# brocksam/pycollo

Hardware: AMD Instinct MI355X
Metric: NLP-callback evals/sec (g + jac_g + hess) (higher is better)
Workload: dtype f64; 1 GPU; hypersensitive, 1 phase, 2000 mesh sections x 6 Lobatto nodes = 10001 collocation nodes; num_x=20003, num_c=10001, nnz_jac=140003, nnz_hess=20002, tiles=167, threads_per_block=64, waves_per_tile=4, launches_per_eval=1, lds_bytes_per_workgroup=24144, launch_thread_cpu=199, pin_survived_hip_init=True

## Files before the change

### __graft_entry__.py

```python
from __future__ import annotations

import os
import subprocess
import sys

ROOT = os.path.dirname(os.path.abspath(__file__))
if ROOT not in sys.path:
    sys.path.insert(0, ROOT)

CSRC = os.path.join(ROOT, "pycollo_amd", "csrc")
LIB = os.path.join(ROOT, "pycollo_amd", "libpycollo_amd.so")


def _run(cmd):
    res = subprocess.run(cmd, capture_output=True, text=True)
    if res.returncode != 0:
        raise RuntimeError(f"{' '.join(cmd)} failed:\n{res.stdout[-2000:]}\n{res.stderr[-4000:]}")


def _stale(target, sources):
    if not os.path.exists(target):
        return True
    t = os.path.getmtime(target)
    return any(os.path.getmtime(s) > t for s in sources)


def build_library(force: bool = False) -> str:
    srcs = [os.path.join(CSRC, f) for f in ("pc_engine.hip", "pc_kkt.hip", "pc_host.hpp", "pc_ipm.hpp", "pc_kkt_cr.hpp", "pc_kkt_shape.hpp", "pc_eval_shape.hpp", "pc_eval_launch.hpp", "pc_pattern.hpp", "pc_desc.hpp", "pc_args.h", "pc_deriv.hpp", "pc_deriv_check.hpp",
                                           "pc_solution_plan.hpp", "pc_costate_plan.hpp", "pc_propagate_plan.hpp",
                                           "pc_solution_host.hpp")]
    srcs.append(os.path.join(ROOT, "include", "pycollo_amd.h"))
    if force or _stale(LIB, srcs):
        hipcc = "/opt/rocm/bin/hipcc" if os.path.exists("/opt/rocm/bin/hipcc") else "hipcc"
        _run([hipcc, "--offload-arch=gfx950", "-O2", "-ffp-contract=off", "-fPIC", "-shared", "-std=c++17", "-o", LIB + ".tmp",
              os.path.join(CSRC, "pc_engine.hip"), os.path.join(CSRC, "pc_kkt.hip")])
        os.replace(LIB + ".tmp", LIB)
    return LIB


PREBUILD = [
    ("brachistochrone", {}, (0,)), ("brachistochrone", {}, (4,)),
    ("hypersensitive", {}, (0,)), ("hypersensitive", {}, (6,)), ("hypersensitive", {}, (5,)), ("hypersensitive", {}, (4,)),
    ("hypersensitive", {}, (2,)), ("hypersensitive", {}, (8,)), ("hypersensitive", {}, (3,)),
    ("hypersensitive", {"fixed_control": 0.0}, (0,)),
    ("cart_pole", {}, (0,)), ("cart_pole", {}, (4,)), ("cart_pole", {}, (5,)),
    ("shuttle", {}, (0,)), ("shuttle", {}, (4,)), ("shuttle", {}, (5,)), ("shuttle", {}, (6,)),
    ("double_pendulum", {}, (0,)), ("double_pendulum", {}, (4,)),
    ("two_phase_transfer", {}, (0, 0)), ("two_phase_transfer", {}, (3, 4)), ("two_phase_transfer", {}, (4, 5)),
    ("two_phase_transfer", {}, (2, 2)), ("two_phase_transfer", {}, (3, 3)), ("two_phase_transfer", {}, (4, 4)),
    ("time_coupled_transfer", {}, (0, 0)), ("time_coupled_transfer", {}, (4, 4)),
    ("time_coupled_transfer", {}, (3, 3)), ("time_coupled_transfer", {}, (3, 4)),
# ... 121 lines not shown
```

### include/pycollo_amd.h

```cpp
#ifndef PYCOLLO_AMD_H
#define PYCOLLO_AMD_H

#include <stdint.h>

#ifdef __cplusplus
extern "C" {
#endif

typedef struct pc_handle pc_handle;

enum { PC_PT_Y0 = 0, PC_PT_YF = 1, PC_PT_Q = 2, PC_PT_T0 = 3, PC_PT_TF = 4, PC_PT_S = 5 };

typedef struct {
  int32_t n_y, n_u, n_q, n_p;
  int32_t t0_free, tF_free;
  double t0_fixed, tF_fixed;
  int32_t K;
  const int32_t* n_k;
  const double* h_k;
  int32_t n_jac;
  const int32_t* jac_row;
  const int32_t* jac_col;
  int32_t n_hess;
  const int32_t* hess_row;
// ... 40 lines not shown
  int32_t device;
  int32_t threads_per_block;
  int32_t two_wave_occupancy;
  int32_t plan_only;
} pc_problem_desc;

typedef struct {
  int32_t n, m;
  int64_t nnz_jac, nnz_hess;
  int64_t algorithmic_bytes;
  int32_t n_tiles_total, threads_per_block;
  int32_t lds_bytes_max, n_launches;
  int32_t waves_per_tile;
  int32_t last_launch;
} pc_info;

#define PC_LAUNCH_RESIDENT 1
#define PC_LAUNCH_TAIL_BIG 2
#define PC_LAUNCH_MERGED 4
#define PC_LAUNCH_TAIL_BLOCKS_SHIFT 4
#define PC_LAUNCH_TAIL_BLOCKS_MASK 7
#define PC_LAUNCH_TAIL_WAVES_SHIFT 8
#define PC_LAUNCH_TAIL_WAVES_MASK 15

const char* pc_last_error(void);

int pc_create(const pc_problem_desc* desc, pc_handle** out);
void pc_destroy(pc_handle* h);
int pc_get_info(const pc_handle* h, pc_info* info);

int pc_sizes(const pc_handle* h, int32_t* n, int32_t* m, int64_t* nnz_jac, int64_t* nnz_hess);
int pc_jac_structure(const pc_handle* h, int32_t* iRow, int32_t* jCol);
int pc_hess_structure(const pc_handle* h, int32_t* iRow, int32_t* jCol);

int pc_set_scaling(pc_handle* h, const double* V_ocp, const double* r_ocp, const double* W_ocp, double w_J);

int pc_eval_f(pc_handle* h, const double* x, int new_x, double* f);
int pc_eval_grad_f(pc_handle* h, const double* x, int new_x, double* grad);
int pc_eval_g(pc_handle* h, const double* x, int new_x, double* g);
int pc_eval_jac_g(pc_handle* h, const double* x, int new_x, double* values);
int pc_eval_h(pc_handle* h, const double* x, int new_x, double obj_factor, const double* lambda,
              int new_lambda, double* values);
int pc_eval_all(pc_handle* h, const double* x, double obj_factor, const double* lambda, double* g,
                double* jac, double* hess);
int pc_ipopt_eval_f(int n, double* x, int new_x, double* obj_value, void* user_data);
int pc_ipopt_eval_grad_f(int n, double* x, int new_x, double* grad_f, void* user_data);
// ... 207 lines not shown
```

### pycollo_amd/csrc/pc_engine.hip

```cpp
#include <hip/hip_runtime.h>

#include <chrono>
#include <cmath>
#include <cstdio>
#include <cstdlib>
#include <cstring>
#include <map>
#include <memory>
#include <string>
#include <vector>

#include "../../include/pycollo_amd.h"
#include "pc_args.h"
#include "pc_host.hpp"
#include "pc_pattern.hpp"
#include "pc_desc.hpp"
#include "pc_eval_shape.hpp"
#include "pc_eval_launch.hpp"
#include "pc_deriv.hpp"
#include "pc_solution_plan.hpp"

struct pc_deriv_dev;
struct pc_kkt;

namespace {

thread_local std::string g_err;

void set_err(const std::string& s) { g_err = s; }

struct PhaseDev {
  DevBuf<int32_t> tile_k0, tile_n0, sec_s;
  DevBuf<double> sec_h, scal, partials, tab;
  DevBuf<int64_t> sec_E, hslot0, hslotN, hsum_slot;
  DevBuf<int32_t> hsum_local;
  DevBuf<unsigned long long> gran;
  hipFunction_t fn = nullptr;
};

__global__ void row_norms_kernel(const int64_t* __restrict__ indptr, const double* __restrict__ val,
                                 double* __restrict__ out, int64_t m) {
// ... 36 lines not shown
}

struct pc_handle : pce::Shape {
  pcp::Problem Q;
  int device = -1;
  bool scaling_set = false;
  std::vector<double> qa, qw;
  hipStream_t stream = nullptr;
  hipModule_t module = nullptr;
  std::vector<hipModule_t> more_modules;
  hipFunction_t fn[pcl::N_KERNELS] = {};
  pcl::Have have;
  pcl::Range rg[PC_MAX_PHASES];
  pcl::Scaling scal;
  pcl::Blocks blocks;
  bool blocks_dirty = true;
  DevBuf<char> d_phase_args;
  DevBuf<PcTileRec> d_trec;
  std::vector<std::unique_ptr<PhaseDev>> pd;
  DevBuf<double> d_qa, d_pointV, d_pointr, d_Wend, d_norms;
  DevBuf<double> d_in, d_out;
  PinBuf<double> h_in, h_out;
  int host_mode = 0;
  hipEvent_t ev_small = nullptr, ev_G = nullptr;
  bool x_valid = false;
  bool fc_valid = false;
  bool small_synced = false, G_synced = false;
  bool prefetch_jac = true;
  bool G_copied = false;
  DevBuf<int64_t> d_point_x, d_tail_owned, d_pt_hslot, d_g_indptr;
  DevBuf<int32_t> d_pt_hlocal;
  DevBuf<unsigned long long> d_erec;
  DevBuf<int64_t> d_rec_slot;
  DevBuf<int32_t> d_rec_term;
  PinBuf<unsigned> h_timeout;
  int spin_us = 500;
  DevBuf<unsigned long long> d_hb_gran;
  PinBuf<double> h_norms;
  std::vector<double> V_ocp, r_ocp, W_ocp;
  int n_launches = 0;
  int last_launch = 0;
  mutable std::shared_ptr<pcd::Plan> deriv_plan;
  std::shared_ptr<pc_deriv_dev> deriv_dev;
};

namespace {

// ... 179 lines not shown
  if (!new_x && h->x_valid) return;
  if (!x) throw std::runtime_error("null x");
  if (x != h->h_in.p) std::memcpy(h->h_in.p, x, h->Q.num_x * sizeof(double));
  if (!(h->host_mode & 1))
    HIP_OK(hipMemcpyAsync(h->d_in.p, h->h_in.p, h->Q.num_x * sizeof(double), hipMemcpyHostToDevice, h->stream));
  h->x_valid = true;
  h->fc_valid = false;
}

void stage_lambda(pc_handle* h, const double* lambda) {
  if (!lambda) throw std::runtime_error("null lambda");
  double* dst = h->h_in.p + h->o_lam;
  if (lambda != dst) std::memcpy(dst, lambda, h->Q.num_c * sizeof(double));
  if (!(h->host_mode & 1))
    HIP_OK(hipMemcpyAsync(h->d_in.p + h->o_lam, dst, h->Q.num_c * sizeof(double), hipMemcpyHostToDevice, h->stream));
}

void copy_down(pc_handle* h, size_t begin, size_t end) {
  if (h->host_mode & 2) return;
  HIP_OK(hipMemcpyAsync(h->h_out.p + begin, h->d_out.p + begin, (end - begin) * sizeof(double), hipMemcpyDeviceToHost,
                        h->stream));
}

hipError_t find_fn(pc_handle* h, hipFunction_t* fn, const char* name) {
  *fn = nullptr;
  hipError_t e = hipModuleGetFunction(fn, h->module, name);
  for (size_t i = 0; e != hipSuccess && i < h->more_modules.size(); ++i) {
    (void)hipGetLastError();
    e = hipModuleGetFunction(fn, h->more_modules[i], name);
  }
  if (e != hipSuccess) *fn = nullptr;
  return e;
}

pce::Knobs read_knobs(int device) {
  pce::Knobs kn;
  auto env_int = [](const char* name, auto& dst) {
    if (const char* env = std::getenv(name)) dst = std::atoi(env);
  };
  auto env_i64 = [](const char* name, int64_t& dst) {
    if (const char* env = std::getenv(name)) dst = std::atoll(env);
  };
  auto env_flag = [](const char* name, bool& dst) {
    if (const char* env = std::getenv(name)) dst = std::atoi(env) != 0;
  };
  env_int("PYCOLLO_AMD_TB", kn.tb);
  env_int("PYCOLLO_AMD_WPT", kn.wpt);
  env_int("PYCOLLO_AMD_TILE_NODES", kn.tile_nodes);
  env_flag("PYCOLLO_AMD_TWO_WAVE", kn.two_wave);
  env_i64("PYCOLLO_AMD_TWO_WAVE_MAX_TILES", kn.two_wave_max_tiles);
  env_i64("PYCOLLO_AMD_TWO_WAVE_TILES", kn.two_wave_tiles);
  env_i64("PYCOLLO_AMD_TWO_WAVE_MAX_WAVES", kn.two_wave_max_waves);
  env_int("PYCOLLO_AMD_MIX_MIN_RUN_ROWS", kn.mix_min_run_rows);
  env_int("PYCOLLO_AMD_MIX_CAP_ROWS", kn.mix_cap_rows);
  env_flag("PYCOLLO_AMD_RESIDENT", kn.resident);
  env_int("PYCOLLO_AMD_TAIL_BLOCKS", kn.tail_blocks);
  env_flag("PYCOLLO_AMD_MERGE", kn.merge);
  int v = 0;
  if (device >= 0 && hipDeviceGetAttribute(&v, hipDeviceAttributeMaxSharedMemoryPerBlock, device) == hipSuccess && v > 0)
    kn.lds_limit = v;
  return kn;
}

}

extern "C" {

const char* pc_last_error(void) { return g_err.c_str(); }

int pc_create(const pc_problem_desc* d, pc_handle** out) {
  if (out) *out = nullptr;
  std::unique_ptr<pc_handle> h;
  const int ok = guarded(g_err, [&] {
    if (!d || !out) throw std::runtime_error("null descriptor or output pointer");
    if (d->n_phases < 1 || d->n_phases > PC_MAX_PHASES) throw std::runtime_error("n_phases must be in [1, 8]");
    h.reset(new pc_handle());
    auto& Q = h->Q;
    pcp::from_desc(*d, Q);
    const pce::Knobs kn = read_knobs(d->device);
    static_cast<pce::Shape&>(*h) = pce::build_shape(*d, Q, kn);
    h->pd.resize(Q.ph.size());
    h->scal.phase.resize(Q.ph.size());
    for (size_t ip = 0; ip < Q.ph.size(); ++ip) {
      h->pd[ip].reset(new PhaseDev());
      h->rg[ip].tile_end = h->ph[ip].n_tiles;
    }
    if (d->plan_only) return;
    h->qa.assign(d->quad_A, d->quad_A + h->qa_n);
    h->qw.assign(d->quad_w, d->quad_w + h->qw_n);
    h->device = d->device;
    h->V_ocp.assign(Q.num_ocp_x, 1.0);
    h->r_ocp.assign(Q.num_ocp_x, 0.0);
    h->W_ocp.assign(Q.num_ocp_c, 1.0);
    if (const char* env = std::getenv("PYCOLLO_AMD_SPIN_US")) h->spin_us = std::atoi(env);
    h->n_launches = pcl::launches_per_evaluation(*h, h->have, Q.ph.size());
    if (h->device < 0) return;

    int ndev = 0;
    if (hipGetDeviceCount(&ndev) != hipSuccess || ndev <= h->device)
      throw std::runtime_error("requested HIP device is not available (no GPU visible?)");
    HIP_OK(hipSetDevice(h->device));
    if (!d->code_object || !d->tail_kernel) throw std::runtime_error("code_object and tail_kernel are required");
    HIP_OK(hipStreamCreateWithFlags(&h->stream, hipStreamNonBlocking));
    HIP_OK(hipModuleLoad(&h->module, d->code_object));
    {
      const std::string path = d->code_object, ext = ".hsaco";
      const std::string base = path.size() > ext.size() && path.compare(path.size() - ext.size(), ext.size(), ext) == 0
                                   ? path.substr(0, path.size() - ext.size()) : path;
      for (int k = 1; k < 16; ++k) {
        const std::string part = base + ".p" + std::to_string(k) + ext;
        FILE* f = std::fopen(part.c_str(), "rb");
        if (!f) break;
        std::fclose(f);
        hipModule_t m = nullptr;
        HIP_OK(hipModuleLoad(&m, part.c_str()));
        h->more_modules.push_back(m);
      }
    }
// ... 43 lines not shown
    {
      std::vector<int64_t> rec_slot(h->rec_slot);
      std::vector<int32_t> rec_term(h->rec_term);
      if (rec_slot.empty()) { rec_slot.push_back(-1); rec_term.push_back(-1); }
      h->d_rec_slot.upload(rec_slot);
      h->d_rec_term.upload(rec_term);
      h->d_erec.upload(std::vector<unsigned long long>(2 * rec_slot.size(), 0ull));
    }
    h->d_hb_gran.upload(std::vector<unsigned long long>(2 * std::max<size_t>(1, Q.pthess_row.size()), 0ull));
    h->h_timeout.alloc(16);
    std::memset(h->h_timeout.p, 0, 16 * sizeof(unsigned));
    h->d_point_x.upload(Q.point_x);
    h->d_tail_owned.upload(Q.tail_owned);
    h->d_pt_hslot.upload(Q.pt_hslot);
    h->d_pt_hlocal.upload(Q.pt_hlocal);
    h->d_g_indptr.upload(Q.g_indptr);
    h->d_in.alloc(h->in_total); h->d_out.alloc(h->out_total);
    h->h_in.alloc(h->in_total); h->h_out.alloc(h->out_total);
    h->d_norms.alloc(Q.num_c); h->h_norms.alloc(Q.num_c);
    HIP_OK(hipMemset(h->d_in.p, 0, h->in_total * sizeof(double)));
    HIP_OK(hipMemset(h->d_out.p, 0, h->out_total * sizeof(double)));
    std::memset(h->h_in.p, 0, h->in_total * sizeof(double));
    std::memset(h->h_out.p, 0, h->out_total * sizeof(double));
    HIP_OK(hipEventCreateWithFlags(&h->ev_small, hipEventDisableTiming));
    HIP_OK(hipEventCreateWithFlags(&h->ev_G, hipEventDisableTiming));
    if (const char* env = std::getenv("PYCOLLO_AMD_HOST_MODE")) h->host_mode = std::atoi(env) & 3;
    h->n_launches = pcl::launches_per_evaluation(*h, h->have, Q.ph.size());
  });
  if (!ok) return 0;
  *out = h.release();
  return 1;
}

void pc_destroy(pc_handle* h) {
  if (!h) return;
  if (h->device >= 0) {
    (void)hipSetDevice(h->device);
    if (h->stream) (void)hipStreamSynchronize(h->stream);
  }
  h->pd.clear();
  if (h->ev_small) (void)hipEventDestroy(h->ev_small);
  if (h->ev_G) (void)hipEventDestroy(h->ev_G);
  for (hipModule_t m : h->more_modules) (void)hipModuleUnload(m);
  if (h->module) (void)hipModuleUnload(h->module);
  if (h->stream) (void)hipStreamDestroy(h->stream);
  delete h;
}

int pc_get_info(const pc_handle* h, pc_info* info) {
  return guarded(g_err, [&] {
    if (!h || !info) throw std::runtime_error("null argument");
    const auto& Q = h->Q;
    info->n = (int32_t)Q.num_x;
    info->m = (int32_t)Q.num_c;
    info->nnz_jac = (int64_t)Q.g_row.size();
    info->nnz_hess = (int64_t)Q.h_row.size();
    info->algorithmic_bytes = 8 * (Q.num_x + Q.num_c) + 8 * (Q.num_c + info->nnz_jac + info->nnz_hess);
    int nt = 0;
    for (auto& D : h->ph) nt += D.n_tiles;
    info->n_tiles_total = nt;
    info->threads_per_block = h->TB;
    info->lds_bytes_max = (h->Q.ph.size() > 1 && h->lds_all > 0) ? h->lds_all : h->lds_max;
    info->n_launches = h->n_launches;
    info->waves_per_tile = 1;
    for (auto& D : h->ph) info->waves_per_tile = std::max(info->waves_per_tile, (int32_t)D.wpt);
    if (h->have.k[pcl::BULK_ALL]) info->waves_per_tile = h->wpt_all;
    info->last_launch = h->last_launch;
  });
}

int pc_sizes(const pc_handle* h, int32_t* n, int32_t* m, int64_t* nnz_jac, int64_t* nnz_hess) {
  return guarded(g_err, [&] {
    if (!h) throw std::runtime_error("null handle");
    if (n) *n = (int32_t)h->Q.num_x;
    if (m) *m = (int32_t)h->Q.num_c;
    if (nnz_jac) *nnz_jac = (int64_t)h->Q.g_row.size();
    if (nnz_hess) *nnz_hess = (int64_t)h->Q.h_row.size();
  });
}

int pc_jac_structure(const pc_handle* h, int32_t* iRow, int32_t* jCol) {
  return guarded(g_err, [&] {
    if (!h || !iRow || !jCol) throw std::runtime_error("null argument");
    std::memcpy(iRow, h->Q.g_row.data(), h->Q.g_row.size() * sizeof(int32_t));
    std::memcpy(jCol, h->Q.g_col.data(), h->Q.g_col.size() * sizeof(int32_t));
  });
}

int pc_hess_structure(const pc_handle* h, int32_t* iRow, int32_t* jCol) {
  return guarded(g_err, [&] {
// ... 132 lines not shown
    auto& P = h->Q.ph[phase];
    for (size_t t = 0; t + 1 < P.tile_k0.size(); ++t) tile_order[t] = t < P.tile_order.size() ? P.tile_order[t] : 0;
  });
}

int pc_set_partials_buffer(pc_handle* h, int phase, double* d_partials) {
  return guarded(g_err, [&] {
    if (!h || phase < 0 || phase >= (int)h->pd.size()) throw std::runtime_error("phase out of range");
    if (h->device >= 0) {
      HIP_OK(hipSetDevice(h->device));
      HIP_OK(hipDeviceSynchronize());
    }
    h->rg[phase].partials_ext = d_partials;
    invalidate_blocks(h);
  });
}

int pc_eval_all(pc_handle* h, const double* x, double obj_factor, const double* lambda, double* g, double* jac,
                double* hess) {
  return guarded(g_err, [&] {
    require_device(h);
    auto& Q = h->Q;
    if (!x || !lambda || !g || !jac || !hess) throw std::runtime_error("null argument");
    if (x != h->h_in.p) std::memcpy(h->h_in.p, x, Q.num_x * sizeof(double));
    if (lambda != h->h_in.p + h->o_lam) std::memcpy(h->h_in.p + h->o_lam, lambda, Q.num_c * sizeof(double));
    if (!(h->host_mode & 1))
      HIP_OK(hipMemcpyAsync(h->d_in.p, h->h_in.p, h->in_total * sizeof(double), hipMemcpyHostToDevice, h->stream));
    pcl::Call call = host_call(h, PC_FLAG_C | PC_FLAG_G | PC_FLAG_H);
    call.sigma = obj_factor;
    launch_all(h, call, h->stream);
    copy_down(h, 0, h->o_H + Q.h_row.size());
    wait_stream(h);
    if (g != h->h_out.p + h->o_c) std::memcpy(g, h->h_out.p + h->o_c, Q.num_c * sizeof(double));
    if (jac != h->h_out.p + h->o_G) std::memcpy(jac, h->h_out.p + h->o_G, Q.g_row.size() * sizeof(double));
    if (hess != h->h_out.p + h->o_H) std::memcpy(hess, h->h_out.p + h->o_H, Q.h_row.size() * sizeof(double));
    h->x_valid = h->fc_valid = h->small_synced = h->G_synced = true;
  });
}

int pc_host_buffers(pc_handle* h, double** x, double** lambda, double** g, double** jac, double** hess) {
  return guarded(g_err, [&] {
    require_device(h);
    if (x) *x = h->h_in.p;
    if (lambda) *lambda = h->h_in.p + h->o_lam;
    if (g) *g = h->h_out.p + h->o_c;
    if (jac) *jac = h->h_out.p + h->o_G;
    if (hess) *hess = h->h_out.p + h->o_H;
  });
}

int pc_set_prefetch_jac(pc_handle* h, int on) {
  return guarded(g_err, [&] {
    require_device(h);
    h->prefetch_jac = on != 0;
  });
}

int pc_set_host_mode(pc_handle* h, int mode) {
  return guarded(g_err, [&] {
    require_device(h);
    if (mode < 0 || mode > 3) throw std::runtime_error("host mode must be 0..3");
    HIP_OK(hipStreamSynchronize(h->stream));
    h->host_mode = mode;
    h->x_valid = h->fc_valid = false;
  });
}

static void ensure_fcG(pc_handle* h, const double* x, int new_x) {
  require_device(h);
  stage_x(h, x, new_x);
  if (h->fc_valid) return;
  launch_all(h, host_call(h, PC_FLAG_C | PC_FLAG_G), h->stream);
  copy_down(h, 0, h->o_c + h->Q.num_c);
  HIP_OK(hipEventRecord(h->ev_small, h->stream));
  h->G_copied = h->prefetch_jac || (h->host_mode & 2);
  if (h->G_copied) {
    copy_down(h, h->o_G, h->o_G + h->Q.g_row.size());
    HIP_OK(hipEventRecord(h->ev_G, h->stream));
  }
  h->fc_valid = true;
  h->small_synced = h->G_synced = false;
}
static void wait_small(pc_handle* h) {
  if (h->small_synced) return;
  if (h->spin_us > 0) {
    const auto t0 = std::chrono::steady_clock::now();
    while (hipEventQuery(h->ev_small) == hipErrorNotReady &&
           std::chrono::duration_cast<std::chrono::microseconds>(std::chrono::steady_clock::now() - t0).count() <= h->spin_us) {}
  }
  HIP_OK(hipEventSynchronize(h->ev_small));
  check_timeout(h);
  h->small_synced = true;
}
static void wait_G(pc_handle* h) {
  if (h->G_synced) return;
  if (!h->G_copied) {
    copy_down(h, h->o_G, h->o_G + h->Q.g_row.size());
    HIP_OK(hipEventRecord(h->ev_G, h->stream));
    h->G_copied = true;
  }
  if (h->spin_us > 0) {
    const auto t0 = std::chrono::steady_clock::now();
    while (hipEventQuery(h->ev_G) == hipErrorNotReady &&
           std::chrono::duration_cast<std::chrono::microseconds>(std::chrono::steady_clock::now() - t0).count() <= h->spin_us) {}
  }
  HIP_OK(hipEventSynchronize(h->ev_G));
  check_timeout(h);
  h->small_synced = h->G_synced = true;
}

int pc_eval_f(pc_handle* h, const double* x, int new_x, double* f) {
  return guarded(g_err, [&] {
    ensure_fcG(h, x, new_x);
    wait_small(h);
    *f = h->h_out.p[h->o_f];
  });
}

int pc_eval_grad_f(pc_handle* h, const double* x, int new_x, double* grad) {
  return guarded(g_err, [&] {
    ensure_fcG(h, x, new_x);
    wait_small(h);
    auto& Q = h->Q;
    std::memset(grad, 0, Q.num_x * sizeof(double));
    for (size_t e = 0; e < Q.jgrad_col.size(); ++e) grad[Q.point_x[Q.jgrad_col[e]]] = h->h_out.p[h->o_gn + e];
  });
}

int pc_eval_g(pc_handle* h, const double* x, int new_x, double* g) {
  return guarded(g_err, [&] {
    ensure_fcG(h, x, new_x);
    wait_small(h);
    if (g != h->h_out.p + h->o_c) std::memcpy(g, h->h_out.p + h->o_c, h->Q.num_c * sizeof(double));
  });
}

int pc_eval_jac_g(pc_handle* h, const double* x, int new_x, double* values) {
  return guarded(g_err, [&] {
    ensure_fcG(h, x, new_x);
    wait_G(h);
    if (values != h->h_out.p + h->o_G) std::memcpy(values, h->h_out.p + h->o_G, h->Q.g_row.size() * sizeof(double));
  });
}

int pc_eval_h(pc_handle* h, const double* x, int new_x, double obj_factor, const double* lambda, int new_lambda,
              double* values) {
  (void)new_lambda;
  return guarded(g_err, [&] {
    require_device(h);
    auto& Q = h->Q;
    stage_x(h, x, new_x);
    stage_lambda(h, lambda);
    pcl::Call call = host_call(h, PC_FLAG_H);
    call.grad_nz = nullptr;
    call.sigma = obj_factor;
    launch_all(h, call, h->stream);
    copy_down(h, h->o_H, h->o_H + Q.h_row.size());
    wait_stream(h);
    h->small_synced = h->fc_valid;
    h->G_synced = h->fc_valid && h->G_copied;
    if (values != h->h_out.p + h->o_H) std::memcpy(values, h->h_out.p + h->o_H, Q.h_row.size() * sizeof(double));
  });
}

int pc_eval_resident(pc_handle* h, const double* x, double obj_factor, const double* lambda, double* f, double* grad,
                     double* g) {
  return guarded(g_err, [&] {
    require_device(h);
    auto& Q = h->Q;
    if (!x) throw std::runtime_error("null x");
    const int mode = h->host_mode;
    h->host_mode = 0;
    try {
      std::memcpy(h->h_in.p, x, Q.num_x * sizeof(double));
      if (lambda) std::memcpy(h->h_in.p + h->o_lam, lambda, Q.num_c * sizeof(double));
      HIP_OK(hipMemcpyAsync(h->d_in.p, h->h_in.p, (lambda ? h->in_total : (size_t)Q.num_x) * sizeof(double),
                            hipMemcpyHostToDevice, h->stream));
      pcl::Call call = host_call(h, PC_FLAG_C | PC_FLAG_G | (lambda ? PC_FLAG_H : 0));
      call.sigma = obj_factor;
      launch_all(h, call, h->stream);
      copy_down(h, 0, h->o_c + Q.num_c);
      wait_stream(h);
    } catch (...) {
      h->host_mode = mode;
// ... 67 lines not shown
int pc_row_norms_jac(pc_handle* h, const double* x, double* norms) {
  return guarded(g_err, [&] {
    require_device(h);
    const int mode = h->host_mode;
    h->host_mode = 0;
    h->x_valid = h->fc_valid = false;
    try {
      ensure_fcG(h, x, 1);
    } catch (...) {
      h->host_mode = mode;
      throw;
    }
    h->host_mode = mode;
    const int64_t m = h->Q.num_c;
    const int64_t threads = m * 64;
    const int blocks = (int)((threads + 255) / 256);
    hipLaunchKernelGGL(row_norms_kernel, dim3(blocks), dim3(256), 0, h->stream, h->d_g_indptr.p, h->d_out.p + h->o_G,
                       h->d_norms.p, m);
    HIP_OK(hipGetLastError());
    HIP_OK(hipMemcpyAsync(h->h_norms.p, h->d_norms.p, m * sizeof(double), hipMemcpyDeviceToHost, h->stream));
    HIP_OK(hipStreamSynchronize(h->stream));
    std::memcpy(norms, h->h_norms.p, m * sizeof(double));
    h->x_valid = h->fc_valid = (mode == 0);
    h->small_synced = h->fc_valid;
    h->G_synced = h->fc_valid && h->G_copied;
  });
}

int pc_interp_linear(int device, const double* tau_prev, int n_prev, const double* vals_prev, int n_vars,
                     const double* tau_new, int n_new, double* out) {
  return guarded(g_err, [&] {
    if (n_prev < 2 || n_new < 1 || n_vars < 0) throw std::runtime_error("interpolation needs at least two abscissae");
    int ndev = 0;
    if (device < 0 || hipGetDeviceCount(&ndev) != hipSuccess || ndev <= device)
      throw std::runtime_error("requested HIP device is not available (no GPU visible?); this library has no CPU fallback");
    HIP_OK(hipSetDevice(device));
    DevBuf<double> d_tp, d_vp, d_tn, d_out;
    d_tp.upload(std::vector<double>(tau_prev, tau_prev + n_prev));
    d_vp.upload(std::vector<double>(vals_prev, vals_prev + (size_t)n_vars * n_prev));
    d_tn.upload(std::vector<double>(tau_new, tau_new + n_new));
    d_out.alloc((size_t)std::max(1, n_vars) * n_new);
    hipLaunchKernelGGL(interp_linear_kernel, dim3((n_new + 255) / 256), dim3(256), 0, 0, d_tp.p, n_prev, d_vp.p, n_vars,
                       d_tn.p, n_new, d_out.p);
    HIP_OK(hipGetLastError());
    HIP_OK(hipMemcpy(out, d_out.p, sizeof(double) * (size_t)n_vars * n_new, hipMemcpyDeviceToHost));
  });
}

// ... 95 lines not shown
```

### pycollo_amd/csrc/pc_eval_shape.hpp

```cpp
#pragma once
#include <algorithm>
#include <cstdint>
#include <map>
#include <optional>
#include <stdexcept>
#include <vector>

#include "pc_args.h"
#include "pc_desc.hpp"
#include "pc_pattern.hpp"

namespace pce {

constexpr int64_t TB128_MIN_NODES = 65536, TB256_MIN_NODES = 262144;
constexpr int64_t ONE_STATE_TB256_MIN_NODES = 25000;
constexpr int HEAVY_EVAL_OPS = 4000;

constexpr int WPT4_MAX_TILES = 400, WPT2_MAX_TILES_HEAVY = 512, WPT2_MAX_TILES = 1024;

constexpr int64_t TWO_WAVE_MIN_TILES64 = 400;
constexpr int QUARTER_CU_LDS = 30 * 1280;
constexpr int64_t TWO_WAVE_TILES = 896;
constexpr int64_t TWO_WAVE_MAX_WAVES = 2048;
constexpr int TWO_WAVE_MIN_TC = 24;
constexpr int TWO_WAVE_MIN_TC_LDS = 32;
constexpr int MIX_CAP_ROWS = 32, MIX_CAP_ROWS_MIN = 8;
constexpr size_t HEAVY_POINT_MIN = 17;
constexpr int TAIL_PARTS = 4;
constexpr int TAIL_BIG_STRIDES = 4;

struct Knobs {
  std::optional<int> tb;
  std::optional<int> wpt;
  std::optional<int> tile_nodes;
  bool two_wave = true;
  int64_t two_wave_max_tiles = 1 << 30;
  int64_t two_wave_tiles = TWO_WAVE_TILES;
  int64_t two_wave_max_waves = TWO_WAVE_MAX_WAVES;
  std::optional<int> mix_min_run_rows;
  int mix_cap_rows = MIX_CAP_ROWS;
  bool resident = true;
  int tail_blocks = 0;
  bool merge = true;
  int lds_limit = 64 * 1024;
};

struct PhaseShape {
  int n_tiles = 0;
  int uni_n = 0, spt = 0;
  int lds_out = 0;
  int lds_out4 = 0;
  bool any_pure = false, any_generic = false;
  int nfs = 0;
  int wpt = 1;
  int lds_bytes = 0;
  int32_t erec0 = 0;
};

struct Shape {
  int TB = 64;
  int TC = 64;
  bool two_wave = false;
  bool mixed = false;
  bool resident = true;
  int lds_limit = 64 * 1024;
  int32_t qa_off[PC_MAX_ORDER + 1], qw_off[PC_MAX_ORDER + 1];
  int qa_n = 0, qw_n = 0;
// ... 309 lines not shown
```

### pycollo_amd/engine.py

```python
from __future__ import annotations

import ctypes as C
import os
from dataclasses import dataclass

import numpy as np
import scipy.sparse as sparse

from . import codegen
from .layout import NlpLayout
from .mesh import PhaseMesh, build_phase_mesh
from .model import Model, compile_model
from .problem import ProblemSpec
from .quadrature import QuadratureTables

_HERE = os.path.dirname(os.path.abspath(__file__))
LIB_PATH = os.path.join(_HERE, "libpycollo_amd.so")

_KIND = {"y0": 0, "yF": 1, "q": 2, "t0": 3, "tF": 4, "s": 5}

_i32p = C.POINTER(C.c_int32)
_f64p = C.POINTER(C.c_double)


# ... 12 lines not shown

class _ProblemDesc(C.Structure):
    _fields_ = [("n_phases", C.c_int32), ("phases", C.POINTER(_PhaseDesc)), ("n_s", C.c_int32),
                ("n_point", C.c_int32), ("point_phase", _i32p), ("point_kind", _i32p), ("point_idx", _i32p),
                ("n_b", C.c_int32),
                ("n_jgrad", C.c_int32), ("jgrad_col", _i32p),
                ("n_bjac", C.c_int32), ("bjac_row", _i32p), ("bjac_col", _i32p),
                ("n_pthess", C.c_int32), ("pthess_row", _i32p), ("pthess_col", _i32p),
                ("n_orders", C.c_int32), ("orders", _i32p), ("quad_A", _f64p), ("quad_w", _f64p),
                ("code_object", C.c_char_p), ("tail_kernel", C.c_char_p),
                ("device", C.c_int32), ("threads_per_block", C.c_int32), ("two_wave_occupancy", C.c_int32),
                ("plan_only", C.c_int32)]


class _Info(C.Structure):
    _fields_ = [("n", C.c_int32), ("m", C.c_int32), ("nnz_jac", C.c_int64), ("nnz_hess", C.c_int64),
                ("algorithmic_bytes", C.c_int64), ("n_tiles_total", C.c_int32), ("threads_per_block", C.c_int32),
                ("lds_bytes_max", C.c_int32), ("n_launches", C.c_int32), ("waves_per_tile", C.c_int32),
                ("last_launch", C.c_int32)]


PC_LAUNCH = dict(RESIDENT=1, TAIL_BIG=2, MERGED=4, TAIL_BLOCKS_SHIFT=4, TAIL_BLOCKS_MASK=7, TAIL_WAVES_SHIFT=8,
                 TAIL_WAVES_MASK=15)


def decode_last_launch(ll: int) -> dict:
    L = PC_LAUNCH
    return dict(resident=bool(ll & L["RESIDENT"]), tail_big=bool(ll & L["TAIL_BIG"]), merged=bool(ll & L["MERGED"]),
                tail_blocks=(ll >> L["TAIL_BLOCKS_SHIFT"]) & L["TAIL_BLOCKS_MASK"],
                tail_block_threads=64 * ((ll >> L["TAIL_WAVES_SHIFT"]) & L["TAIL_WAVES_MASK"]))


class _DerivEntry(C.Structure):
    _fields_ = [("kind", C.c_int32), ("located", C.c_int32), ("index", C.c_int64), ("row", C.c_int64), ("col", C.c_int64),
                ("analytic", C.c_double), ("fd", C.c_double), ("err", C.c_double)]


PC_DERIV_MAX_REPORT = 64


class _DerivOpts(C.Structure):
    _fields_ = [("tol", C.c_double), ("delta", C.c_double), ("max_report", C.c_int32), ("reserved", C.c_int32),
                ("seed", C.c_uint64), ("d_jgrad_override", C.c_void_p), ("d_jac_fd", C.c_void_p),
                ("d_hess_fd", C.c_void_p), ("d_jgrad_fd", C.c_void_p)]


# ... 296 lines not shown
        desc.n_bjac, desc.bjac_row, desc.bjac_col = len(br), _ptr(br, _i32p), _ptr(bc, _i32p)
        desc.n_pthess, desc.pthess_row, desc.pthess_col = len(phr), _ptr(phr, _i32p), _ptr(phc, _i32p)
        desc.n_orders, desc.orders, desc.quad_A, desc.quad_w = len(orders), _ptr(od, _i32p), _ptr(qa, _f64p), _ptr(qw, _f64p)
        desc.code_object = code_object.encode() if code_object else None
        desc.tail_kernel = b"pc_tail"
        desc.device = self.device
        desc.threads_per_block = int(tpb)
        desc.two_wave_occupancy = codegen.two_wave_occupancy(m, code_object) if code_object else 0
        return desc

    def _check(self, ok):
        if not ok:
            raise RuntimeError(self._lib.pc_last_error().decode())

    @property
    def info(self) -> dict:
        if not self._h:
            return dict(self._info_closed)
        info = _Info()
        self._check(self._lib.pc_get_info(self._h, C.byref(info)))
        out = {k: getattr(info, k) for k, _ in _Info._fields_}
        ll = out["last_launch"]
        out.update(decode_last_launch(ll))
        return out

    def close(self):
        if getattr(self, "_h", None) is not None and self._h:
            self._info_closed = self.info
            self._lib.pc_destroy(self._h)
            self._h = C.c_void_p()

    def __del__(self):
        try:
            self.close()
        except Exception:
            pass

    def set_scaling(self, V_ocp, r_ocp, W_ocp, w_J: float = 1.0):
        self.V_ocp = np.ascontiguousarray(V_ocp, dtype=np.float64)
        self.r_ocp = np.ascontiguousarray(r_ocp, dtype=np.float64)
        self.W_ocp = np.ascontiguousarray(W_ocp, dtype=np.float64)
        self.w_J = float(w_J)
        if self.V_ocp.shape != (self.layout.num_ocp_x,) or self.r_ocp.shape != (self.layout.num_ocp_x,):
            raise ValueError(f"V_ocp / r_ocp must have {self.layout.num_ocp_x} entries")
        if self.W_ocp.shape != (self.layout.num_ocp_c,):
            raise ValueError(f"W_ocp must have {self.layout.num_ocp_c} entries")
# ... 327 lines not shown
```

Before: 236,100 evals/s.

## Chunk device-to-host output copies and overlap with host memcpy delivery

Splits the device-to-host copy of the output buffer (constraints, Jacobian, Hessian) into up to 16 chunks of about 448 KiB, each with its own event. The host then copies each chunk into the caller's arrays as soon as that chunk arrives, rather than waiting for the whole transfer to finish. When there are more than two chunks, it also alternates them across a second stream so two DMA transfers can run at once. The aim is to hide the host memcpy and part of the transfer latency, at the cost of more events, more API calls and extra synchronisation logic.

```diff
diff --git a/__graft_entry__.py b/__graft_entry__.py
--- a/__graft_entry__.py
+++ b/__graft_entry__.py
@@ -26,7 +26,7 @@
 
 
 def build_library(force: bool = False) -> str:
-    srcs = [os.path.join(CSRC, f) for f in ("pc_engine.hip", "pc_kkt.hip", "pc_host.hpp", "pc_ipm.hpp", "pc_kkt_cr.hpp", "pc_kkt_shape.hpp", "pc_eval_shape.hpp", "pc_eval_launch.hpp", "pc_pattern.hpp", "pc_desc.hpp", "pc_args.h", "pc_deriv.hpp", "pc_deriv_check.hpp",
+    srcs = [os.path.join(CSRC, f) for f in ("pc_engine.hip", "pc_kkt.hip", "pc_host.hpp", "pc_ipm.hpp", "pc_kkt_cr.hpp", "pc_kkt_shape.hpp", "pc_eval_shape.hpp", "pc_eval_launch.hpp", "pc_deliver.hpp", "pc_pattern.hpp", "pc_desc.hpp", "pc_args.h", "pc_deriv.hpp", "pc_deriv_check.hpp",
                                            "pc_solution_plan.hpp", "pc_costate_plan.hpp", "pc_propagate_plan.hpp",
                                            "pc_solution_host.hpp")]
     srcs.append(os.path.join(ROOT, "include", "pycollo_amd.h"))
diff --git a/include/pycollo_amd.h b/include/pycollo_amd.h
--- a/include/pycollo_amd.h
+++ b/include/pycollo_amd.h
@@ -86,6 +86,8 @@
 #define PC_LAUNCH_TAIL_BLOCKS_MASK 7
 #define PC_LAUNCH_TAIL_WAVES_SHIFT 8
 #define PC_LAUNCH_TAIL_WAVES_MASK 15
+#define PC_DELIVER_CHUNKS_SHIFT 16
+#define PC_DELIVER_CHUNKS_MASK 255
 
 const char* pc_last_error(void);
 
diff --git a/pycollo_amd/csrc/pc_deliver.hpp b/pycollo_amd/csrc/pc_deliver.hpp
--- /dev/null
+++ b/pycollo_amd/csrc/pc_deliver.hpp
@@ -0,0 +1,97 @@
+#pragma once
+#include <algorithm>
+#include <cstddef>
+#include <cstdint>
+
+namespace pcv {
+
+constexpr size_t GRAIN = 32;
+constexpr int MAX_CHUNKS = 16;
+constexpr int N_ARRAYS = 3;
+constexpr int64_t DEFAULT_CHUNK_BYTES = 448 * 1024;
+
+struct Layout {
+  size_t o_f = 0, o_gn = 1, n_gn = 0;
+  size_t off[N_ARRAYS] = {0, 0, 0};
+  size_t len[N_ARRAYS] = {0, 0, 0};
+  size_t small_end() const { return off[1]; }
+  size_t end() const { return off[2] + len[2]; }
+};
+
+struct Dest {
+  double* p[N_ARRAYS] = {nullptr, nullptr, nullptr};
+};
+
+struct Copy {
+  double* dst = nullptr;
+  size_t src_begin = 0, count = 0;
+};
+
+struct Chunk {
+  size_t begin = 0, end = 0;
+  int n_copies = 0;
+  Copy copy[N_ARRAYS];
+};
+
+struct Plan {
+  int n = 0;
+  Chunk c[MAX_CHUNKS];
+};
+
+inline bool needs_copy(const Layout& L, size_t begin, size_t end, const Dest& d, const double* staging) {
+  for (int a = 0; a < N_ARRAYS; ++a)
+    if (d.p[a] && d.p[a] != staging + L.off[a] && std::max(begin, L.off[a]) < std::min(end, L.off[a] + L.len[a])) return true;
+  return false;
+}
+
+inline void cut(const Layout& L, size_t begin, size_t end, size_t chunk_bytes, int cap, Plan& P) {
+  P.n = 0;
+  end = std::min(end, L.end());
+  if (begin >= end) return;
+  cap = std::min(std::max(cap, 1), MAX_CHUNKS);
+  size_t S = chunk_bytes / sizeof(double) / GRAIN * GRAIN;
+  if (chunk_bytes > 0 && S == 0) S = GRAIN;
+  auto push = [&](size_t b, size_t e) {
+    P.c[P.n].begin = b;
+    P.c[P.n].end = e;
+    P.c[P.n].n_copies = 0;
+    ++P.n;
+  };
+  if (S == 0 || cap == 1) {
+    push(begin, end);
+    return;
+  }
+  size_t from = begin;
+  if (begin < L.small_end() && end > L.small_end()) {
+    from = L.small_end();
+    push(begin, from);
+  }
+  const size_t base = from / GRAIN * GRAIN, room = (size_t)(cap - P.n);
+  if ((end - base + S - 1) / S > room) S = ((end - base + room - 1) / room + GRAIN - 1) / GRAIN * GRAIN;
+  for (size_t b = base; b < end; b += S) push(std::max(b, from), std::min(b + S, end));
+}
+
+inline void bind(const Layout& L, const Dest& d, const double* staging, Plan& P) {
+  for (int i = 0; i < P.n; ++i) {
+    Chunk& c = P.c[i];
+    c.n_copies = 0;
+    for (int a = 0; a < N_ARRAYS; ++a) {
+      if (!d.p[a] || d.p[a] == staging + L.off[a]) continue;
+      const size_t lo = std::max(c.begin, L.off[a]), hi = std::min(c.end, L.off[a] + L.len[a]);
+      if (lo >= hi) continue;
+      Copy& r = c.copy[c.n_copies++];
+      r.dst = d.p[a] + (lo - L.off[a]);
+      r.src_begin = lo;
+      r.count = hi - lo;
+    }
+  }
+}
+
+inline Plan plan(const Layout& L, size_t begin, size_t end, const Dest& d, const double* staging, size_t chunk_bytes, int cap) {
+  Plan P;
+  cut(L, begin, end, needs_copy(L, begin, end, d, staging) ? chunk_bytes : 0, cap, P);
+  bind(L, d, staging, P);
+  return P;
+}
+
+}
diff --git a/pycollo_amd/csrc/pc_engine.hip b/pycollo_amd/csrc/pc_engine.hip
--- a/pycollo_amd/csrc/pc_engine.hip
+++ b/pycollo_amd/csrc/pc_engine.hip
@@ -17,6 +17,7 @@
 #include "pc_desc.hpp"
 #include "pc_eval_shape.hpp"
 #include "pc_eval_launch.hpp"
+#include "pc_deliver.hpp"
 #include "pc_deriv.hpp"
 #include "pc_solution_plan.hpp"
 
@@ -99,7 +100,14 @@
   DevBuf<double> d_in, d_out;
   PinBuf<double> h_in, h_out;
   int host_mode = 0;
-  hipEvent_t ev_small = nullptr, ev_G = nullptr;
+  pcv::Layout lay;
+  size_t deliver_chunk = pcv::DEFAULT_CHUNK_BYTES;
+  hipEvent_t ev[pcv::MAX_CHUNKS] = {};
+  pcv::Plan fc;
+  int fc_done = 0;
+  hipStream_t stream2 = nullptr;
+  hipEvent_t ev_launch = nullptr;
+  int last_chunks = 0;
   bool x_valid = false;
   bool fc_valid = false;
   bool small_synced = false, G_synced = false;
@@ -325,6 +333,56 @@
                         h->stream));
 }
 
+void copy_down(pc_handle* h, const pcv::Plan& P, int first, bool drain) {
+  for (int i = first; i < P.n; ++i) {
+    copy_down(h, P.c[i].begin, P.c[i].end);
+    if (!(drain && i == P.n - 1)) HIP_OK(hipEventRecord(h->ev[i], h->stream));
+  }
+  h->last_chunks = P.n;
+}
+
+bool two_streams(const pc_handle* h, const pcv::Plan& P) { return h->stream2 && P.n > 2 && !(h->host_mode & 2); }
+void copy_down_two_streams(pc_handle* h, const pcv::Plan& P) {
+  HIP_OK(hipEventRecord(h->ev_launch, h->stream));
+  HIP_OK(hipStreamWaitEvent(h->stream2, h->ev_launch, 0));
+  for (int i = 0; i < P.n; ++i) {
+    hipStream_t st = (i & 1) ? h->stream2 : h->stream;
+    HIP_OK(hipMemcpyAsync(h->h_out.p + P.c[i].begin, h->d_out.p + P.c[i].begin, (P.c[i].end - P.c[i].begin) * sizeof(double),
+                          hipMemcpyDeviceToHost, st));
+    HIP_OK(hipEventRecord(h->ev[i], st));
+  }
+  h->last_chunks = P.n;
+}
+
+void wait_event(pc_handle* h, hipEvent_t ev) {
+  if (h->spin_us > 0) {
+    const auto t0 = std::chrono::steady_clock::now();
+    while (hipEventQuery(ev) == hipErrorNotReady &&
+           std::chrono::duration_cast<std::chrono::microseconds>(std::chrono::steady_clock::now() - t0).count() <= h->spin_us) {}
+  }
+  HIP_OK(hipEventSynchronize(ev));
+}
+
+void deliver(pc_handle* h, const pcv::Plan& P, int arrived, int upto, bool drain) {
+  for (int i = 0; i < upto; ++i) {
+    const pcv::Chunk& c = P.c[i];
+    if (i >= arrived) {
+      if (drain && i == P.n - 1) wait_stream(h);
+      else wait_event(h, h->ev[i]);
+    }
+    for (int r = 0; r < c.n_copies; ++r) std::memcpy(c.copy[r].dst, h->h_out.p + c.copy[r].src_begin, c.copy[r].count * sizeof(double));
+  }
+  if (upto > arrived) check_timeout(h);
+}
+
+size_t chunk_bytes(const pc_handle* h) { return (h->host_mode & 2) ? 0 : h->deliver_chunk; }
+
+void fc_arrived(pc_handle* h) {
+  h->small_synced = h->fc_valid;
+  h->G_synced = h->fc_valid && h->G_copied;
+  h->fc_done = h->fc_valid ? h->fc.n : 0;
+}
+
 hipError_t find_fn(pc_handle* h, hipFunction_t* fn, const char* name) {
   *fn = nullptr;
   hipError_t e = hipModuleGetFunction(fn, h->module, name);
@@ -359,6 +417,8 @@
   env_flag("PYCOLLO_AMD_RESIDENT", kn.resident);
   env_int("PYCOLLO_AMD_TAIL_BLOCKS", kn.tail_blocks);
   env_flag("PYCOLLO_AMD_MERGE", kn.merge);
+  env_i64("PYCOLLO_AMD_DELIVER_CHUNK", kn.deliver_chunk);
+  env_int("PYCOLLO_AMD_DELIVER_STREAMS", kn.deliver_streams);
   int v = 0;
   if (device >= 0 && hipDeviceGetAttribute(&v, hipDeviceAttributeMaxSharedMemoryPerBlock, device) == hipSuccess && v > 0)
     kn.lds_limit = v;
@@ -397,6 +457,10 @@
     h->W_ocp.assign(Q.num_ocp_c, 1.0);
     if (const char* env = std::getenv("PYCOLLO_AMD_SPIN_US")) h->spin_us = std::atoi(env);
     h->n_launches = pcl::launches_per_evaluation(*h, h->have, Q.ph.size());
+    h->deliver_chunk = (size_t)std::max<int64_t>(0, kn.deliver_chunk);
+    h->lay.o_f = h->o_f; h->lay.o_gn = h->o_gn; h->lay.n_gn = Q.jgrad_col.size();
+    h->lay.off[0] = h->o_c; h->lay.off[1] = h->o_G; h->lay.off[2] = h->o_H;
+    h->lay.len[0] = Q.num_c; h->lay.len[1] = Q.g_row.size(); h->lay.len[2] = Q.h_row.size();
     if (h->device < 0) return;
 
     int ndev = 0;
@@ -486,8 +550,11 @@
     HIP_OK(hipMemset(h->d_out.p, 0, h->out_total * sizeof(double)));
     std::memset(h->h_in.p, 0, h->in_total * sizeof(double));
     std::memset(h->h_out.p, 0, h->out_total * sizeof(double));
-    HIP_OK(hipEventCreateWithFlags(&h->ev_small, hipEventDisableTiming));
-    HIP_OK(hipEventCreateWithFlags(&h->ev_G, hipEventDisableTiming));
+    for (hipEvent_t& e : h->ev) HIP_OK(hipEventCreateWithFlags(&e, hipEventDisableTiming));
+    if (kn.deliver_streams >= 2) {
+      HIP_OK(hipStreamCreateWithFlags(&h->stream2, hipStreamNonBlocking));
+      HIP_OK(hipEventCreateWithFlags(&h->ev_launch, hipEventDisableTiming));
+    }
     if (const char* env = std::getenv("PYCOLLO_AMD_HOST_MODE")) h->host_mode = std::atoi(env) & 3;
     h->n_launches = pcl::launches_per_evaluation(*h, h->have, Q.ph.size());
   });
@@ -503,10 +570,15 @@
     if (h->stream) (void)hipStreamSynchronize(h->stream);
   }
   h->pd.clear();
-  if (h->ev_small) (void)hipEventDestroy(h->ev_small);
-  if (h->ev_G) (void)hipEventDestroy(h->ev_G);
+  for (hipEvent_t e : h->ev)
+    if (e) (void)hipEventDestroy(e);
   for (hipModule_t m : h->more_modules) (void)hipModuleUnload(m);
   if (h->module) (void)hipModuleUnload(h->module);
+  if (h->stream2) {
+    (void)hipStreamSynchronize(h->stream2);
+    (void)hipStreamDestroy(h->stream2);
+  }
+  if (h->ev_launch) (void)hipEventDestroy(h->ev_launch);
   if (h->stream) (void)hipStreamDestroy(h->stream);
   delete h;
 }
@@ -529,7 +601,7 @@
     info->waves_per_tile = 1;
     for (auto& D : h->ph) info->waves_per_tile = std::max(info->waves_per_tile, (int32_t)D.wpt);
     if (h->have.k[pcl::BULK_ALL]) info->waves_per_tile = h->wpt_all;
-    info->last_launch = h->last_launch;
+    info->last_launch = h->last_launch | (h->last_chunks & PC_DELIVER_CHUNKS_MASK) << PC_DELIVER_CHUNKS_SHIFT;
   });
 }
 
@@ -708,6 +780,7 @@
     require_device(h);
     auto& Q = h->Q;
     if (!x || !lambda || !g || !jac || !hess) throw std::runtime_error("null argument");
+    h->x_valid = h->fc_valid = h->small_synced = h->G_synced = false;
     if (x != h->h_in.p) std::memcpy(h->h_in.p, x, Q.num_x * sizeof(double));
     if (lambda != h->h_in.p + h->o_lam) std::memcpy(h->h_in.p + h->o_lam, lambda, Q.num_c * sizeof(double));
     if (!(h->host_mode & 1))
@@ -715,12 +788,17 @@
     pcl::Call call = host_call(h, PC_FLAG_C | PC_FLAG_G | PC_FLAG_H);
     call.sigma = obj_factor;
     launch_all(h, call, h->stream);
-    copy_down(h, 0, h->o_H + Q.h_row.size());
-    wait_stream(h);
-    if (g != h->h_out.p + h->o_c) std::memcpy(g, h->h_out.p + h->o_c, Q.num_c * sizeof(double));
-    if (jac != h->h_out.p + h->o_G) std::memcpy(jac, h->h_out.p + h->o_G, Q.g_row.size() * sizeof(double));
-    if (hess != h->h_out.p + h->o_H) std::memcpy(hess, h->h_out.p + h->o_H, Q.h_row.size() * sizeof(double));
-    h->x_valid = h->fc_valid = h->small_synced = h->G_synced = true;
+    pcv::Dest dst;
+    dst.p[0] = g; dst.p[1] = jac; dst.p[2] = hess;
+    const pcv::Plan P = pcv::plan(h->lay, 0, h->lay.end(), dst, h->h_out.p, chunk_bytes(h), pcv::MAX_CHUNKS);
+    const bool two = two_streams(h, P);
+    if (two) copy_down_two_streams(h, P);
+    else copy_down(h, P, 0, true);
+    deliver(h, P, 0, P.n, !two);
+    pcv::cut(h->lay, 0, h->lay.off[1] + h->lay.len[1], 0, 1, h->fc);
+    h->G_copied = true;
+    h->x_valid = h->fc_valid = true;
+    fc_arrived(h);
   });
 }
 
@@ -752,53 +830,55 @@
   });
 }
 
+static void copy_down_G(pc_handle* h) {
+  const pcv::Layout& L = h->lay;
+  pcv::Plan G;
+  pcv::cut(L, L.off[1], L.off[1] + L.len[1], chunk_bytes(h), pcv::MAX_CHUNKS - h->fc.n, G);
+  const int first = h->fc.n;
+  for (int i = 0; i < G.n; ++i) h->fc.c[h->fc.n++] = G.c[i];
+  copy_down(h, h->fc, first, false);
+}
 static void ensure_fcG(pc_handle* h, const double* x, int new_x) {
   require_device(h);
   stage_x(h, x, new_x);
   if (h->fc_valid) return;
+  h->small_synced = h->G_synced = false;
+  h->fc_done = 0;
   launch_all(h, host_call(h, PC_FLAG_C | PC_FLAG_G), h->stream);
-  copy_down(h, 0, h->o_c + h->Q.num_c);
-  HIP_OK(hipEventRecord(h->ev_small, h->stream));
+  pcv::cut(h->lay, 0, h->lay.off[0] + h->lay.len[0], 0, 1, h->fc);
+  copy_down(h, h->fc, 0, false);
   h->G_copied = h->prefetch_jac || (h->host_mode & 2);
-  if (h->G_copied) {
-    copy_down(h, h->o_G, h->o_G + h->Q.g_row.size());
-    HIP_OK(hipEventRecord(h->ev_G, h->stream));
-  }
+  if (h->G_copied) copy_down_G(h);
   h->fc_valid = true;
-  h->small_synced = h->G_synced = false;
-}
-static void wait_small(pc_handle* h) {
-  if (h->small_synced) return;
-  if (h->spin_us > 0) {
-    const auto t0 = std::chrono::steady_clock::now();
-    while (hipEventQuery(h->ev_small) == hipErrorNotReady &&
-           std::chrono::duration_cast<std::chrono::microseconds>(std::chrono::steady_clock::now() - t0).count() <= h->spin_us) {}
-  }
-  HIP_OK(hipEventSynchronize(h->ev_small));
-  check_timeout(h);
-  h->small_synced = true;
-}
-static void wait_G(pc_handle* h) {
-  if (h->G_synced) return;
+}
+static void deliver_fc(pc_handle* h, int upto, const pcv::Dest& dst) {
+  const int arrived = h->fc_done;
+  if (upto > arrived) h->small_synced = h->G_synced = false, h->fc_done = 0;
+  pcv::bind(h->lay, dst, h->h_out.p, h->fc);
+  deliver(h, h->fc, arrived, upto, false);
+  h->fc_done = std::max(arrived, upto);
+  h->small_synced = h->fc_done >= 1;
+  h->G_synced = h->G_copied && h->fc_done == h->fc.n;
+}
+static void deliver_small(pc_handle* h, double* g) {
+  pcv::Dest dst;
+  dst.p[0] = g;
+  deliver_fc(h, 1, dst);
+}
+static void deliver_G(pc_handle* h, double* values) {
   if (!h->G_copied) {
-    copy_down(h, h->o_G, h->o_G + h->Q.g_row.size());
-    HIP_OK(hipEventRecord(h->ev_G, h->stream));
+    copy_down_G(h);
     h->G_copied = true;
   }
-  if (h->spin_us > 0) {
-    const auto t0 = std::chrono::steady_clock::now();
-    while (hipEventQuery(h->ev_G) == hipErrorNotReady &&
-           std::chrono::duration_cast<std::chrono::microseconds>(std::chrono::steady_clock::now() - t0).count() <= h->spin_us) {}
-  }
-  HIP_OK(hipEventSynchronize(h->ev_G));
-  check_timeout(h);
-  h->small_synced = h->G_synced = true;
+  pcv::Dest dst;
+  dst.p[1] = values;
+  deliver_fc(h, h->fc.n, dst);
 }
 
 int pc_eval_f(pc_handle* h, const double* x, int new_x, double* f) {
   return guarded(g_err, [&] {
     ensure_fcG(h, x, new_x);
-    wait_small(h);
+    deliver_small(h, nullptr);
     *f = h->h_out.p[h->o_f];
   });
 }
@@ -806,7 +886,7 @@
 int pc_eval_grad_f(pc_handle* h, const double* x, int new_x, double* grad) {
   return guarded(g_err, [&] {
     ensure_fcG(h, x, new_x);
-    wait_small(h);
+    deliver_small(h, nullptr);
     auto& Q = h->Q;
     std::memset(grad, 0, Q.num_x * sizeof(double));
     for (size_t e = 0; e < Q.jgrad_col.size(); ++e) grad[Q.point_x[Q.jgrad_col[e]]] = h->h_out.p[h->o_gn + e];
@@ -816,16 +896,14 @@
 int pc_eval_g(pc_handle* h, const double* x, int new_x, double* g) {
   return guarded(g_err, [&] {
     ensure_fcG(h, x, new_x);
-    wait_small(h);
-    if (g != h->h_out.p + h->o_c) std::memcpy(g, h->h_out.p + h->o_c, h->Q.num_c * sizeof(double));
+    deliver_small(h, g);
   });
 }
 
 int pc_eval_jac_g(pc_handle* h, const double* x, int new_x, double* values) {
   return guarded(g_err, [&] {
     ensure_fcG(h, x, new_x);
-    wait_G(h);
-    if (values != h->h_out.p + h->o_G) std::memcpy(values, h->h_out.p + h->o_G, h->Q.g_row.size() * sizeof(double));
+    deliver_G(h, values);
   });
 }
 
@@ -834,18 +912,23 @@
   (void)new_lambda;
   return guarded(g_err, [&] {
     require_device(h);
-    auto& Q = h->Q;
     stage_x(h, x, new_x);
     stage_lambda(h, lambda);
     pcl::Call call = host_call(h, PC_FLAG_H);
     call.grad_nz = nullptr;
     call.sigma = obj_factor;
     launch_all(h, call, h->stream);
-    copy_down(h, h->o_H, h->o_H + Q.h_row.size());
-    wait_stream(h);
-    h->small_synced = h->fc_valid;
-    h->G_synced = h->fc_valid && h->G_copied;
-    if (values != h->h_out.p + h->o_H) std::memcpy(values, h->h_out.p + h->o_H, Q.h_row.size() * sizeof(double));
+    pcv::Dest dst;
+    dst.p[2] = values;
+    const pcv::Plan P = pcv::plan(h->lay, h->lay.off[2], h->lay.end(), dst, h->h_out.p, chunk_bytes(h), pcv::MAX_CHUNKS);
+    const bool fc_was = h->fc_valid;
+    h->fc_valid = h->small_synced = h->G_synced = false;
+    h->fc_done = 0;
+    copy_down(h, P, 0, true);
+    deliver(h, P, 0, P.n, true);
+    if (P.n == 0) wait_stream(h);
+    h->fc_valid = fc_was;
+    fc_arrived(h);
   });
 }
 
@@ -959,8 +1042,7 @@
     HIP_OK(hipStreamSynchronize(h->stream));
     std::memcpy(norms, h->h_norms.p, m * sizeof(double));
     h->x_valid = h->fc_valid = (mode == 0);
-    h->small_synced = h->fc_valid;
-    h->G_synced = h->fc_valid && h->G_copied;
+    fc_arrived(h);
   });
 }
 
diff --git a/pycollo_amd/csrc/pc_eval_shape.hpp b/pycollo_amd/csrc/pc_eval_shape.hpp
--- a/pycollo_amd/csrc/pc_eval_shape.hpp
+++ b/pycollo_amd/csrc/pc_eval_shape.hpp
@@ -7,6 +7,7 @@
 #include <vector>
 
 #include "pc_args.h"
+#include "pc_deliver.hpp"
 #include "pc_desc.hpp"
 #include "pc_pattern.hpp"
 
@@ -43,6 +44,8 @@
   int tail_blocks = 0;
   bool merge = true;
   int lds_limit = 64 * 1024;
+  int64_t deliver_chunk = pcv::DEFAULT_CHUNK_BYTES;
+  int deliver_streams = 2;
 };
 
 struct PhaseShape {
diff --git a/pycollo_amd/engine.py b/pycollo_amd/engine.py
--- a/pycollo_amd/engine.py
+++ b/pycollo_amd/engine.py
@@ -58,6 +58,9 @@
 
 PC_LAUNCH = dict(RESIDENT=1, TAIL_BIG=2, MERGED=4, TAIL_BLOCKS_SHIFT=4, TAIL_BLOCKS_MASK=7, TAIL_WAVES_SHIFT=8,
                  TAIL_WAVES_MASK=15)
+
+
+PC_DELIVER_CHUNKS_SHIFT, PC_DELIVER_CHUNKS_MASK = 16, 255
 
 
 def decode_last_launch(ll: int) -> dict:
@@ -400,6 +403,8 @@
         out = {k: getattr(info, k) for k, _ in _Info._fields_}
         ll = out["last_launch"]
         out.update(decode_last_launch(ll))
+        out["deliver_chunks"] = (ll >> PC_DELIVER_CHUNKS_SHIFT) & PC_DELIVER_CHUNKS_MASK
+        out["last_launch"] = ll & ~(PC_DELIVER_CHUNKS_MASK << PC_DELIVER_CHUNKS_SHIFT)
         return out
 
     def close(self):
```

After: 240,500 evals/s (median of 4 runs). Within noise of the previous version (+1.9%).
